# AnneLouisedb/dlwp-benchmark

Measured on AMD Instinct MI355X. Metric: rollout cell-steps/s, higher is better.
Workload: dtype f32 (f16x3: products from two-part f16 splits, 22-bit operands, fp32 accumulate)

## Files before the change

dlwp_benchmark_amd/csrc/fno2d.hip:

```cpp
#include "common.hpp"
#include "spectral_any.hpp"
#include <atomic>
#include <memory>

#ifndef DLWP_GELU8_LIFT
#define DLWP_GELU8_LIFT gelu_erf8
#endif
#ifndef DLWP_GELU8_PROJ
#define DLWP_GELU8_PROJ gelu_erf8
#endif
#ifndef DLWP_GELU8_TRUNK
#define DLWP_GELU8_TRUNK gelu_erf8
#endif

namespace dlwp {
namespace fno {

constexpr int kC = 32;
constexpr int kTrStride = 68;

struct ChanSeg {
  const float* ptr;
  long long bstride;
  int nchan;
// ... 873 lines not shown
        const int c = 4 * s + g;
        *reinterpret_cast<f32x4*>(s_tr + c * kTrStride + 4 * j) =
            *reinterpret_cast<const f32x4*>(x + ((long long)b * kC + c) * HW + pix);
      }
      wave_lds_fence();
      fwd_dft_accumulate<2, KP>(s_tr, tt, w0, lane, yacc);
      wave_lds_fence();
    }
    store_y<2, KP>(ybuf, row, kC, lane, yacc);
  }
}

struct ModesParams {
  const float* ybuf;
  float* zbuf;
  const float2* wt;
  const float2* ef;
  const float2* ei;
  const float* ck;
  float fwd_scale;
  int B, H, M1, M2, KP;
};

__device__ __forceinline__ float2 cfma(float2 a, float2 b, float2 c) {
  return float2{fmaf(a.x, b.x, fmaf(-a.y, b.y, c.x)), fmaf(a.x, b.y, fmaf(a.y, b.x, c.y))};
}

template <int HC, int RG>
__global__ __launch_bounds__(1024) void fno_modes_kernel(const ModesParams p) {
  extern __shared__ __align__(16) float smem[];
  constexpr int C = kC, CP = 32 / RG, CN = C / CP;
  const int ky = blockIdx.x, b = blockIdx.y, tid = threadIdx.x;
  const int lo = tid & 31, hi = tid >> 5;
  const int H = p.H, M1 = p.M1, KP = p.KP;
  float* zb = p.zbuf + (long long)b * H * KP * C;
  if (ky >= p.M2) {
    for (int i = tid; i < H * C; i += 1024) {
      const int o = i & 31, h = i >> 5;
      zb[((long long)h * KP + 2 * ky) * C + o] = 0.f;
      zb[((long long)h * KP + 2 * ky + 1) * C + o] = 0.f;
    }
    return;
  }
  float2* s_ef = reinterpret_cast<float2*>(smem);
  float2* s_ei = s_ef + M1 * H;
  float2* s_part = s_ei + M1 * H;
  float2* s_x = s_part + 16 * M1 * C;
  float2* s_o = s_x + M1 * C;

  float2 yv[HC];
  {
    const float* yb = p.ybuf + (long long)b * H * KP * C;
#pragma unroll
    for (int i = 0; i < HC; ++i) {
      const int h = hi * HC + i;
      if (h < H) {
        yv[i].x = yb[((long long)h * KP + 2 * ky) * C + lo];
        yv[i].y = yb[((long long)h * KP + 2 * ky + 1) * C + lo];
      } else {
        yv[i] = float2{0.f, 0.f};
      }
    }
  }
  for (int i = tid; i < M1 * H; i += 1024) {
    s_ef[i] = p.ef[i];
    s_ei[i] = p.ei[i];
  }
  const int r2 = hi % RG, cpart = hi / RG;
  float2 wreg[CN];
  {
    const float2* w = p.wt + ((long long)ky * M1 + (r2 < M1 ? r2 : 0)) * C * C + (size_t)cpart * CN * C + lo;
#pragma unroll
    for (int c = 0; c < CN; ++c) wreg[c] = w[c * C];
  }
  __syncthreads();
  for (int r = 0; r < M1; ++r) {
    float2 acc = {0.f, 0.f};
#pragma unroll
    for (int i = 0; i < HC; ++i) {
      const int h = hi * HC + i;
      acc = cfma(yv[i], s_ef[r * H + (h < H ? h : 0)], acc);
    }
    acc.x += __shfl_xor(acc.x, 32);
    acc.y += __shfl_xor(acc.y, 32);
    if ((tid & 32) == 0) s_part[((tid >> 6) * M1 + r) * C + lo] = acc;
  }
  __syncthreads();
  for (int i = tid; i < M1 * C; i += 1024) {
    float2 a = s_part[i];
#pragma unroll
    for (int w = 1; w < 16; ++w) {
      const float2 t = s_part[w * M1 * C + i];
      a.x += t.x;
      a.y += t.y;
    }
    s_x[i] = float2{a.x * p.fwd_scale, a.y * p.fwd_scale};
  }
  __syncthreads();
  if (r2 < M1) {
    float2 acc = {0.f, 0.f};
#pragma unroll
    for (int c = 0; c < CN; ++c) acc = cfma(s_x[r2 * C + cpart * CN + c], wreg[c], acc);
    s_part[(cpart * M1 + r2) * C + lo] = acc;
  }
  __syncthreads();
  for (int i = tid; i < M1 * C; i += 1024) {
    float2 a = s_part[i];
#pragma unroll
    for (int cp = 1; cp < CP; ++cp) {
      const float2 t = s_part[cp * M1 * C + i];
      a.x += t.x;
      a.y += t.y;
    }
    s_o[i] = a;
  }
  __syncthreads();
  {
    float2 acc[HC];
#pragma unroll
    for (int i = 0; i < HC; ++i) acc[i] = float2{0.f, 0.f};
    for (int r = 0; r < M1; ++r) {
      const float2 ov = s_o[r * C + lo];
#pragma unroll
      for (int i = 0; i < HC; ++i) {
        const int h = hi * HC + i;
        acc[i] = cfma(ov, s_ei[r * H + (h < H ? h : 0)], acc[i]);
      }
    }
    const float ck = p.ck[ky];
#pragma unroll
    for (int i = 0; i < HC; ++i) {
      const int h = hi * HC + i;
      if (h < H) {
        zb[((long long)h * KP + 2 * ky) * C + lo] = acc[i].x * ck;
        zb[((long long)h * KP + 2 * ky + 1) * C + lo] = acc[i].y * ck;
      }
    }
  }
}

constexpr int kTrunkMaxLayers = 8;
#ifndef DLWP_TRUNK_DFT_BF16
#define DLWP_TRUNK_DFT_BF16 0
#endif
constexpr bool kDftBf16 = DLWP_TRUNK_DFT_BF16 != 0;
#ifndef DLWP_F16_DFT
#define DLWP_F16_DFT 1
#endif
#ifndef DLWP_PREFETCH_EARLY
#define DLWP_PREFETCH_EARLY 0
#endif
constexpr int kTrunkF16Shift = 3;
constexpr float kTrunkF16Up = 16384.0f, kTrunkF16Down = 1.0f / 16384.0f;
constexpr int kSyStride = 528;

struct TrunkParams {
  const float* x;
  float* y;
  const float* ybuf;
  const float* t;
  const float* tt;
  const u32x4* tb;
  const u32x4* ttb;
  const float2* ef;
  const float2* ei;
  const float* ck;
  const u32x4* wsb[kTrunkMaxLayers];
  const float* bias[kTrunkMaxLayers];
  const float2* wt[kTrunkMaxLayers];
  float* xpart;
  float* obuf;
  long long xpart_par, obuf_par;
  unsigned layer0;
  unsigned* xcc_tab;
  unsigned* ctr;
  unsigned epoch;
  float fwd_scale;
  int S, H, L, M1, M2, G, sample0;
  unsigned long long* trace;
  int trace_tid;
  ChanTable in;
  int lift_ns, lift_hid;
  int lift_cin1;
  const float* lift_w1p;
  const float* lift_b1;
  const u32x4* lift_w2b;
  const float* lift_b2;
  const float* lift_tab;
  float lift_up, lift_down, proj_up, proj_down;
  int proj_hid, proj_co, cout;
  const u32x4* proj_w1b;
  const float* proj_b1;
  const float* proj_w2v;
  const float* proj_b2;
  float* out;
  long long out_bstride;
  const float* resid;
  long long resid_bstride;
  const float* r_const;
  const float* r_presc;
  const float* r_prog;
  float* r_out;
  int r_nconst, r_npresc, r_nprog, r_T, r_ctx, r_t0;
  int feed_regs;
  int n_steps;
  int spin_limit, try_limit;
  unsigned* fail_word;
  unsigned* sticky_fails;
};

__device__ __forceinline__ void trunk_group_barrier(unsigned* ctr, unsigned target, int* s_fail, int spin_limit) {
  __builtin_amdgcn_fence(__ATOMIC_RELEASE, "workgroup");
  __builtin_amdgcn_s_waitcnt(0);
  __syncthreads();
  if (threadIdx.x == 0) {
    __hip_atomic_fetch_add(ctr, 1u, __ATOMIC_RELAXED, __HIP_MEMORY_SCOPE_AGENT);
    int spins = 0;
    while ((int)(__hip_atomic_load(ctr, __ATOMIC_RELAXED, __HIP_MEMORY_SCOPE_AGENT) - target) < 0) {
      __builtin_amdgcn_s_sleep(1);
      if (++spins > spin_limit) {
        *s_fail = 1;
        break;
      }
    }
  }
  __syncthreads();
}

__device__ __forceinline__ void trunk_group_arrive(unsigned* ctr) {
  __builtin_amdgcn_fence(__ATOMIC_RELEASE, "workgroup");
  __builtin_amdgcn_s_waitcnt(0);
  __syncthreads();
  if (threadIdx.x == 0) __hip_atomic_fetch_add(ctr, 1u, __ATOMIC_RELAXED, __HIP_MEMORY_SCOPE_AGENT);
}
__device__ __forceinline__ void trunk_group_wait(unsigned* ctr, unsigned target, int* s_fail, int spin_limit) {
  if (threadIdx.x == 0) {
    int spins = 0;
    while ((int)(__hip_atomic_load(ctr, __ATOMIC_RELAXED, __HIP_MEMORY_SCOPE_AGENT) - target) < 0) {
      __builtin_amdgcn_s_sleep(1);
      if (++spins > spin_limit) {
        *s_fail = 1;
        break;
      }
    }
  }
  __syncthreads();
}

__device__ __forceinline__ float ld_sc1(const float* p) {
  return __hip_atomic_load(p, __ATOMIC_RELAXED, __HIP_MEMORY_SCOPE_AGENT);
}
__device__ __forceinline__ void st_sc1(float* p, float v) {
  __hip_atomic_store(p, v, __ATOMIC_RELAXED, __HIP_MEMORY_SCOPE_AGENT);
}

__device__ __forceinline__ void ld4_sc1_x4(const float* base, unsigned o0, unsigned o1, unsigned o2, unsigned o3,
                                           f32x4& v0, f32x4& v1, f32x4& v2, f32x4& v3) {
  asm volatile(
      "s_nop 4\n\t"
      "global_load_dwordx4 %0, %4, %8 sc1\n\t"
      "global_load_dwordx4 %1, %5, %8 sc1\n\t"
      "global_load_dwordx4 %2, %6, %8 sc1\n\t"
      "global_load_dwordx4 %3, %7, %8 sc1\n\t"
      "s_waitcnt vmcnt(0)"
      : "=&v"(v0), "=&v"(v1), "=&v"(v2), "=&v"(v3)
      : "v"(o0), "v"(o1), "v"(o2), "v"(o3), "s"(base)
      : "memory");
}
constexpr unsigned kSentinel = 0x7fc0deadu;
__device__ __forceinline__ bool has_sentinel(const f32x4& v) {
  return __float_as_uint(v[0]) == kSentinel || __float_as_uint(v[1]) == kSentinel ||
         __float_as_uint(v[2]) == kSentinel || __float_as_uint(v[3]) == kSentinel;
}
__device__ __forceinline__ void st4_sc1(const float* base, unsigned off, const f32x4& v) {
  asm volatile("s_nop 4\n\tglobal_store_dwordx4 %0, %1, %2 sc1\n\ts_nop 1" : : "v"(off), "v"(v), "s"(base) : "memory");
}
__device__ __forceinline__ void st4_l2(const float* base, unsigned off, const f32x4& v) {
  asm volatile("s_nop 4\n\tglobal_store_dwordx4 %0, %1, %2\n\ts_nop 1" : : "v"(off), "v"(v), "s"(base) : "memory");
}
__device__ __forceinline__ void st_xchg(float* p, float v, bool fast) {
  if (fast) *p = v;
  else __hip_atomic_store(p, v, __ATOMIC_RELAXED, __HIP_MEMORY_SCOPE_AGENT);
}

__device__ __forceinline__ void lds_barrier() {
  asm volatile("s_waitcnt lgkmcnt(0)\n\ts_barrier" ::: "memory");
}
__device__ __forceinline__ f32x4 shfl_xor4(f32x4 v, int m) {
  return f32x4{__shfl_xor(v[0], m), __shfl_xor(v[1], m), __shfl_xor(v[2], m), __shfl_xor(v[3], m)};
}

__device__ __forceinline__ void rollout_step_io(const TrunkParams& p, int t, long long HW, ChanTable& in, float*& out,
                                                long long& out_bs, const float*& resid, long long& resid_bs) {
  const int T = p.r_T, ctx = p.r_ctx, To = T - ctx;
  const long long prog_bs = (long long)T * p.r_nprog * HW;
  out_bs = (long long)To * p.r_nprog * HW;
  int k = 0;
#pragma unroll
  for (int i = 0; i < 4; ++i) in.seg[i] = ChanSeg{nullptr, 0, 0, 0};
  if (p.r_nconst) in.seg[k++] = ChanSeg{p.r_const, (long long)p.r_nconst * HW, p.r_nconst, 0};
  if (p.r_npresc)
    in.seg[k++] = ChanSeg{p.r_presc + (long long)(t - ctx) * p.r_npresc * HW, (long long)T * p.r_npresc * HW, p.r_npresc * ctx, 0};
  const int f0 = t - ctx;
  const int n_in = (f0 < ctx) ? (ctx - f0 < ctx ? ctx - f0 : ctx) : 0;
  if (n_in > 0) in.seg[k++] = ChanSeg{p.r_prog + (long long)f0 * p.r_nprog * HW, prog_bs, p.r_nprog * n_in, 0};
  if (ctx - n_in > 0) {
    const int fo = f0 + n_in - ctx;
    in.seg[k++] = ChanSeg{p.r_out + (long long)fo * p.r_nprog * HW, out_bs, p.r_nprog * (ctx - n_in), 0};
  }
  if (t - 1 < ctx) { resid = p.r_prog + (long long)(t - 1) * p.r_nprog * HW; resid_bs = prog_bs; }
  else { resid = p.r_out + (long long)(t - 1 - ctx) * p.r_nprog * HW; resid_bs = out_bs; }
  out = p.r_out + (long long)(t - ctx) * p.r_nprog * HW;
}

template <bool F16 = false>
__device__ __forceinline__ void fwd_dft_bf16x6(const float* s_tr, const u32x4* s_ttb, int lane, f32x4 (&yacc)[2]) {
  const int j = lane & 15, g = lane >> 4;
#pragma unroll
  for (int kb = 0; kb < 2; ++kb) {
    u32x4 tb[3];
#pragma unroll
    for (int pp = 0; pp < 3; ++pp) tb[pp] = s_ttb[(kb * 3 + pp) * 64 + lane];
#pragma unroll
    for (int ct = 0; ct < 2; ++ct) {
      const float* src = s_tr + (16 * ct + j) * kTrStride + 32 * kb + 8 * g;
      const f32x4 a0 = *reinterpret_cast<const f32x4*>(src), a1 = *reinterpret_cast<const f32x4*>(src + 4);
      u32x4 xa[3];
#pragma unroll
      for (int i = 0; i < 4; ++i) {
        unsigned hh, mm, ll;
        const float v0 = i < 2 ? a0[2 * i] : a1[2 * i - 4], v1 = i < 2 ? a0[2 * i + 1] : a1[2 * i - 3];
        split_pair_x<F16>(v0, v1, hh, mm, ll);
        xa[0][i] = hh;
        xa[1][i] = mm;
        xa[2][i] = ll;
      }
      if constexpr (F16) {
        yacc[ct] = mfma16x16x32_f16(xa[0], tb[1], yacc[ct]);
        yacc[ct] = mfma16x16x32_f16(xa[1], tb[0], yacc[ct]);
        yacc[ct] = mfma16x16x32_f16(xa[0], tb[2], yacc[ct]);
      } else {
        yacc[ct] = mfma_bf16x6(xa, tb, yacc[ct]);
      }
    }
  }
}

template <int ROWS, int G, bool LL, bool STEP = false, bool F16 = false>
__global__ __launch_bounds__(64 * ROWS, 2) void fno_trunk_kernel(const TrunkParams p) {
  extern __shared__ __align__(16) float smem[];
  constexpr int W = 64, KP = 16, C = kC, NT = 64 * ROWS;
  constexpr bool kDftF16 = F16 && (DLWP_F16_DFT != 0);
  static_assert(!F16 || kDftF16, "f16x3: the skip convolution and the inverse W-DFT share one SCALED accumulator (common.hpp)");
  constexpr bool kDftMx = kDftBf16 || kDftF16;
  const int tid = threadIdx.x, lane = tid & 63, wave = tid >> 6;
  const int j = lane & 15, g = lane >> 4;
  float* s_tr = smem + wave * (C * kTrStride);
  float* s_y = smem + ROWS * C * kTrStride;
  float* s_z = s_y + ROWS * kSyStride;
  float* s_x = s_z + ROWS * KP * C;
  float* s_t = s_x + ROWS * 128;
  float* s_tt = s_t + KP * W;
  int* s_fail = reinterpret_cast<int*>(s_tt + W * KP);
  int* s_fast = s_fail + 1;
  float2* s_ef = reinterpret_cast<float2*>(s_fail + 4);
  float2* s_ei = s_ef + 16 * ROWS;
  u32x4* s_tb = reinterpret_cast<u32x4*>(s_ei + 16 * ROWS);
  u32x4* s_ttb = s_tb + 4 * 3 * 64;
  const int H = p.H, M1 = p.M1, M2 = p.M2, NM = M1 * M2;
  int sample, member;
  {
    const int i = blockIdx.x;
    if ((p.S & 7) == 0) {
      const int slot = i >> 3;
      sample = (i & 7) + 8 * (slot / G);
      member = slot % G;
    } else {
      sample = i / G;
      member = i % G;
    }
  }
  const int h = member * ROWS + wave;
  const long long HW = (long long)H * W;
  const int gs = p.sample0 + sample;
  const long long pix = (long long)h * W + 4 * j;
  unsigned* ctr = p.ctr + sample * 32;
  if (tid == 0) {
    *s_fail = 0;
    *s_fast = 0;
    if (LL) {
      const unsigned xcc = __builtin_amdgcn_s_getreg((20 << 0) | (0 << 6) | (31 << 11)) & 0xFu;
      __hip_atomic_store(p.xcc_tab + sample * 32 + member, ((p.layer0 + 1u) << 4) | xcc, __ATOMIC_RELAXED,
                         __HIP_MEMORY_SCOPE_AGENT);
    }
  }
  for (int i = tid; i < ROWS * KP * C; i += NT) s_z[i] = 0.f;
  for (int i = tid; i < KP * W; i += NT) {
    s_t[i] = p.t[i];
    s_tt[i] = p.tt[i];
  }
  for (int i = tid; i < 16 * ROWS; i += NT) {
    const int r = i / ROWS, hl = i % ROWS;
    s_ef[i] = r < M1 ? p.ef[r * H + member * ROWS + hl] : float2{0.f, 0.f};
    s_ei[i] = r < M1 ? p.ei[r * H + member * ROWS + hl] : float2{0.f, 0.f};
  }
  for (int i = tid; i < 4 * 3 * 64; i += NT) s_tb[i] = p.tb[i];
  for (int i = tid; i < 2 * 3 * 64; i += NT) s_ttb[i] = p.ttb[i];
  lds_barrier();

  int n_stamp = 0;
  const int n_steps = (STEP && p.n_steps > 1) ? p.n_steps : 1;
  f32x4 vfeed = {0.f, 0.f, 0.f, 0.f};
  u32x4 pre_w2[6];
  float pre_w1[8], pre_b1 = 0.f;
  bool staged = false;
  for (int st = 0; st < n_steps; ++st) {
  int tid_o = threadIdx.x;
  asm volatile("" : "+v"(tid_o));
  const int tid = tid_o, lane = tid & 63, wave = tid >> 6, j = lane & 15, g = lane >> 4;
  float* s_tr = smem + wave * (C * kTrStride);
  const int h = member * ROWS + wave;
  const long long pix = (long long)h * W + 4 * j;
  ChanTable in = p.in;
  float* out_p = p.out;
  long long out_bs = p.out_bstride, resid_bs = p.resid_bstride;
  const float* resid_p = p.resid;
  if (STEP && p.n_steps > 1) rollout_step_io(p, p.r_t0 + st, HW, in, out_p, out_bs, resid_p, resid_bs);
  f32x4 vv[2][4];
  if constexpr (STEP) {
    if (p.trace && tid == p.trace_tid && n_stamp < 64) p.trace[blockIdx.x * 64 + n_stamp++] = __builtin_amdgcn_s_memrealtime();
    const int ntile_l = p.lift_hid >> 4, npair = ntile_l >> 1;
    u32x4* l_w2 = reinterpret_cast<u32x4*>(smem);
    float* l_w1 = reinterpret_cast<float*>(l_w2 + npair * 6 * 64);
    float* l_b1 = l_w1 + ntile_l * p.lift_ns * 64;
    if (!staged) {
      for (int i = tid; i < npair * 6 * 64; i += NT) l_w2[i] = p.lift_w2b[i];
      for (int i = tid; i < ntile_l * p.lift_ns * 64; i += NT) l_w1[i] = p.lift_w1p[i];
      for (int i = tid; i < p.lift_hid; i += NT) l_b1[i] = p.lift_b1[i];
    }
    f32x4 xs[4];
    if (p.feed_regs && st > 0) {
      xs[0] = vfeed;
#pragma unroll
      for (int s = 1; s < 4; ++s) xs[s] = f32x4{0.f, 0.f, 0.f, 0.f};
    } else {
#pragma unroll
      for (int s = 0; s < 4; ++s) {
        const float* cp = s < p.lift_ns ? chan_ptr(in, 4 * s + g, gs, (int)HW) : nullptr;
        xs[s] = cp ? *reinterpret_cast<const f32x4*>(cp + pix) : f32x4{0.f, 0.f, 0.f, 0.f};
      }
    }
    f32x4 bias2[2];
    bias2[0] = *reinterpret_cast<const f32x4*>(p.lift_b2 + 4 * g);
    bias2[1] = *reinterpret_cast<const f32x4*>(p.lift_b2 + 16 + 4 * g);
    lds_barrier();
    if (p.trace && tid == p.trace_tid && n_stamp < 64) p.trace[blockIdx.x * 64 + n_stamp++] = __builtin_amdgcn_s_memrealtime();
    bool from_table = false;
    f32x4 xp = {0.f, 0.f, 0.f, 0.f};
#ifndef DLWP_NO_LIFT_TABLE
    if (p.lift_tab) {
      bool inside = true;
#pragma unroll
      for (int q = 0; q < 4; ++q) {
        xp[q] = __shfl(xs[0][q], lane >> 2);
        inside = inside && (fabsf(xp[q]) < (float)kLiftTabRange);
      }
      from_table = __all(inside) != 0;
    }
#endif
    if (from_table) {
      f32x4 vp[2][4];
      lift_from_table(p.lift_tab, xp, lane & 3, vp);
#pragma unroll
      for (int ot = 0; ot < 2; ++ot)
#pragma unroll
        for (int r = 0; r < 4; ++r)
#pragma unroll
          for (int q = 0; q < 4; ++q) vv[ot][r][q] = __shfl(vp[ot][r][q], 4 * j + g);
    } else {
      f32x4 acc2[2][4];
      lift_segment<4, F16>(xs, l_w1, l_b1, l_w2, npair, lane, bias2, acc2, p.lift_ns, p.lift_cin1 != 0, p.lift_up, p.lift_down);
#pragma unroll
      for (int ot = 0; ot < 2; ++ot)
#pragma unroll
        for (int r = 0; r < 4; ++r) vv[ot][r] = f32x4{acc2[ot][0][r], acc2[ot][1][r], acc2[ot][2][r], acc2[ot][3][r]};
    }
    if (p.trace && tid == p.trace_tid && n_stamp < 64) p.trace[blockIdx.x * 64 + n_stamp++] = __builtin_amdgcn_s_memrealtime();
    lds_barrier();
    if (p.trace && tid == p.trace_tid && n_stamp < 64) p.trace[blockIdx.x * 64 + n_stamp++] = __builtin_amdgcn_s_memrealtime();
#pragma unroll
    for (int ot = 0; ot < 2; ++ot)
#pragma unroll
      for (int r = 0; r < 4; ++r)
        *reinterpret_cast<f32x4*>(s_tr + (16 * ot + 4 * g + r) * kTrStride + 4 * j) = vv[ot][r];
    wave_lds_fence();
    f32x4 yacc[2] = {f32x4{0.f, 0.f, 0.f, 0.f}, f32x4{0.f, 0.f, 0.f, 0.f}};
    if constexpr (kDftMx) {
      fwd_dft_bf16x6<kDftF16>(s_tr, s_ttb, lane, yacc);
    } else {
#pragma unroll
      for (int s = 0; s < 16; ++s)
#pragma unroll
        for (int ct = 0; ct < 2; ++ct)
          yacc[ct] = mfma16x16x4(s_tr[(16 * ct + j) * kTrStride + 4 * s + g], s_tt[(4 * s + g) * KP + j], yacc[ct]);
    }
    wave_lds_fence();
#pragma unroll
    for (int ct = 0; ct < 2; ++ct)
      *reinterpret_cast<f32x4*>(s_y + wave * kSyStride + j * C + 16 * ct + 4 * g) = kDftF16 ? yacc[ct] * kTrunkF16Down : yacc[ct];
    if (p.trace && tid == p.trace_tid && n_stamp < 64) p.trace[blockIdx.x * 64 + n_stamp++] = __builtin_amdgcn_s_memrealtime();
  } else {
#pragma unroll
    for (int ot = 0; ot < 2; ++ot)
#pragma unroll
      for (int r = 0; r < 4; ++r)
        vv[ot][r] = *reinterpret_cast<const f32x4*>(p.x + ((long long)gs * C + 16 * ot + 4 * g + r) * HW + pix);
    const float* yr = p.ybuf + ((long long)gs * H + h) * KP * C;
#pragma unroll
    for (int u = 0; u < 2; ++u)
      *reinterpret_cast<f32x4*>(s_y + wave * kSyStride + 4 * lane + 256 * u) =
          *reinterpret_cast<const f32x4*>(yr + 4 * lane + 256 * u);
  }
  constexpr int KS1 = ROWS / 2;
  float a_re[KS1], a_im[KS1];
#pragma unroll
  for (int s = 0; s < KS1; ++s) {
    const int hl = 2 * s + (g >> 1);
    float2 e = {0.f, 0.f};
    if (j < M1) e = s_ef[j * ROWS + hl];
    a_re[s] = (g & 1) ? -e.y : e.x;
    a_im[s] = (g & 1) ? e.x : e.y;
  }
  float a3[8];
#pragma unroll
  for (int s = 0; s < 8; ++s) {
    const int r = 2 * s + (g >> 1);
    float2 e = {0.f, 0.f};
    if (r < M1 && (j >> 1) < ROWS) e = s_ei[r * ROWS + (j >> 1)];
    a3[s] = (j & 1) ? ((g & 1) ? e.x : e.y) : ((g & 1) ? -e.y : e.x);
  }
  const int ks3 = (2 * M1 + 3) / 4;
  const int per = (NM + G - 1) / G;
  const int m_lo = member * per, m_hi = (m_lo + per < NM) ? m_lo + per : NM;
  float* xp_mine0 = p.xpart + ((long long)sample * G + member) * NM * 64;
  const float* xp_grp0 = p.xpart + (long long)sample * G * NM * 64;
  float* ob0 = p.obuf + (long long)sample * NM * 64;
  unsigned target = p.epoch * (unsigned)G;

#define DLWP_STAMP()                                                                                   \
  do {                                                                                                 \
    if (p.trace && tid == p.trace_tid && n_stamp < 64) p.trace[blockIdx.x * 64 + n_stamp++] = __builtin_amdgcn_s_memrealtime(); \
  } while (0)
  DLWP_STAMP();

  for (int l = 0; l < p.L; ++l) {
    const int par = LL ? (int)((p.layer0 + (unsigned)(st * p.L + l)) & 1u) : 0;
    float* xp_mine = xp_mine0 + par * p.xpart_par;
    const float* xp_grp = xp_grp0 + par * p.xpart_par;
    float* ob = ob0 + par * p.obuf_par;
    float* ob_other = ob0 + (par ^ 1) * p.obuf_par;
    if (LL) asm volatile("s_waitcnt vmcnt(0)" ::: "memory");
    const bool fast = LL && (l > 0 || st > 0) && (*s_fast != 0);
    u32x4 wb[2][3];
#pragma unroll
    for (int ot = 0; ot < 2; ++ot)
#pragma unroll
      for (int pp = 0; pp < 3; ++pp) wb[ot][pp] = p.wsb[l][(ot * 3 + pp) * 64 + lane];
    f32x4 bias4[2];
#pragma unroll
    for (int ot = 0; ot < 2; ++ot) bias4[ot] = *reinterpret_cast<const f32x4*>(p.bias[l] + 16 * ot + 4 * g);
    float2 wreg[2][16];
    {
      const int m = m_lo + wave;
      const float2* w = p.wt[l] + ((long long)(m < m_hi ? m : 0) * C + (lane >> 5) * 16) * C + (lane & 31);
#pragma unroll
      for (int cc = 0; cc < 16; ++cc) wreg[0][cc] = w[cc * C];
    }
    lds_barrier();
    DLWP_STAMP();
    for (int ky = wave; ky < M2; ky += ROWS) {
      f32x4 dre[2] = {f32x4{0.f, 0.f, 0.f, 0.f}, f32x4{0.f, 0.f, 0.f, 0.f}}, dim[2] = {dre[0], dre[0]};
#pragma unroll
      for (int s = 0; s < KS1; ++s) {
#pragma unroll
        for (int nt = 0; nt < 2; ++nt) {
          const float b = s_y[(2 * s + (g >> 1)) * kSyStride + (2 * ky + (g & 1)) * C + 16 * nt + j];
          dre[nt] = mfma16x16x4(a_re[s], b, dre[nt]);
          dim[nt] = mfma16x16x4(a_im[s], b, dim[nt]);
        }
      }
      auto publish = [&](auto fastc) {
        constexpr bool FAST = decltype(fastc)::value;
#pragma unroll
        for (int nt = 0; nt < 2; ++nt)
#pragma unroll
          for (int r4 = 0; r4 < 4; ++r4) {
            const int r = 4 * g + r4;
            if (r < M1) {
              float* dst = xp_mine + (long long)(ky * M1 + r) * 64 + 16 * nt + j;
              if constexpr (!LL) {
                st_sc1(dst, dre[nt][r4]);
                st_sc1(dst + 32, dim[nt][r4]);
              } else if constexpr (FAST) {
                dst[0] = dre[nt][r4];
                dst[32] = dim[nt][r4];
              } else {
                __hip_atomic_store(dst, dre[nt][r4], __ATOMIC_RELAXED, __HIP_MEMORY_SCOPE_AGENT);
                __hip_atomic_store(dst + 32, dim[nt][r4], __ATOMIC_RELAXED, __HIP_MEMORY_SCOPE_AGENT);
              }
            }
          }
      };
      if (fast) publish(std::true_type{}); else publish(std::false_type{});
    }
    DLWP_STAMP();
    target += (unsigned)G;
    if (!LL) trunk_group_arrive(ctr);
    f32x4 acc[2][4];
#pragma unroll
    for (int ot = 0; ot < 2; ++ot)
#pragma unroll
      for (int q = 0; q < 4; ++q) acc[ot][q] = F16 ? bias4[ot] * kTrunkF16Up : bias4[ot];
#pragma unroll
    for (int q = 0; q < 4; ++q) {
      u32x4 bx[3];
#pragma unroll
      for (int i = 0; i < 4; ++i) {
        unsigned hh, mm, ll;
        split_pair_x<F16>(vv[i >> 1][2 * (i & 1)][q], vv[i >> 1][2 * (i & 1) + 1][q], hh, mm, ll);
        bx[0][i] = hh;
        bx[1][i] = mm;
        bx[2][i] = ll;
      }
#pragma unroll
      for (int ot = 0; ot < 2; ++ot) acc[ot][q] = mfma_x<F16>(wb[ot], bx, acc[ot][q]);
    }
    if (!LL) trunk_group_wait(ctr, target, s_fail, p.spin_limit);
    DLWP_STAMP();
    {
      const int m = m_lo + wave + ROWS;
      const float2* w = p.wt[l] + ((long long)(m < m_hi ? m : 0) * C + (lane >> 5) * 16) * C + (lane & 31);
#pragma unroll
// ... 151 lines not shown
            s_z[(2 * g + (r4 >> 1)) * (KP * C) + (kDftMx ? o * KP + kq : kq * C + o)] = d[r4] * ckw;
          }
      }
      wave_lds_fence();
    }
    lds_barrier();
    DLWP_STAMP();
    if constexpr (kDftMx) {
      u32x4 za[2][3];
#pragma unroll
      for (int ot = 0; ot < 2; ++ot) {
        f32x4 z0 = {0.f, 0.f, 0.f, 0.f}, z1 = z0;
        if (g < 2) {
          const float* src = s_z + wave * (KP * C) + (16 * ot + j) * KP + 8 * g;
          z0 = *reinterpret_cast<const f32x4*>(src);
          z1 = *reinterpret_cast<const f32x4*>(src + 4);
        }
#pragma unroll
        for (int i = 0; i < 4; ++i) {
          unsigned hh, mm, ll;
          const float v0 = i < 2 ? z0[2 * i] : z1[2 * i - 4], v1 = i < 2 ? z0[2 * i + 1] : z1[2 * i - 3];
          split_pair_x<kDftF16>(v0, v1, hh, mm, ll);
          za[ot][0][i] = hh;
          za[ot][1][i] = mm;
          za[ot][2][i] = ll;
        }
      }
#pragma unroll
      for (int q = 0; q < 4; ++q) {
        u32x4 tb[3];
#pragma unroll
        for (int pp = 0; pp < 3; ++pp) tb[pp] = s_tb[(q * 3 + pp) * 64 + lane];
#pragma unroll
        for (int ot = 0; ot < 2; ++ot) {
          if constexpr (kDftF16) {
            acc[ot][q] = mfma16x16x32_f16(za[ot][0], tb[1], acc[ot][q]);
            acc[ot][q] = mfma16x16x32_f16(za[ot][1], tb[0], acc[ot][q]);
            acc[ot][q] = mfma16x16x32_f16(za[ot][0], tb[2], acc[ot][q]);
          } else {
            acc[ot][q] = mfma_bf16x6(za[ot], tb, acc[ot][q]);
          }
        }
      }
    } else {
      float z[KP / 4][2];
#pragma unroll
      for (int s = 0; s < KP / 4; ++s)
#pragma unroll
        for (int ot = 0; ot < 2; ++ot) z[s][ot] = s_z[wave * (KP * C) + (4 * s + g) * C + 16 * ot + j];
#pragma unroll
      for (int s = 0; s < KP / 4; ++s) {
        const f32x4 tw = *reinterpret_cast<const f32x4*>(s_t + (4 * s + g) * W + 4 * j);
#pragma unroll
        for (int q = 0; q < 4; ++q)
#pragma unroll
          for (int ot = 0; ot < 2; ++ot) acc[ot][q] = mfma16x16x4(z[s][ot], tw[q], acc[ot][q]);
      }
    }
#pragma unroll
    for (int ot = 0; ot < 2; ++ot)
#pragma unroll
      for (int r = 0; r < 4; ++r) {
        vv[ot][r] = f32x4{acc[ot][0][r], acc[ot][1][r], acc[ot][2][r], acc[ot][3][r]};
        if constexpr (F16) vv[ot][r] *= kTrunkF16Down;
      }
    DLWP_STAMP();
    if (l < p.L - 1) {
#pragma unroll
      for (int ot = 0; ot < 2; ++ot) {
        DLWP_GELU8_TRUNK(vv[ot][0], vv[ot][1]);
        DLWP_GELU8_TRUNK(vv[ot][2], vv[ot][3]);
      }
      DLWP_STAMP();
#pragma unroll
      for (int ot = 0; ot < 2; ++ot)
#pragma unroll
        for (int r = 0; r < 4; ++r)
          *reinterpret_cast<f32x4*>(s_tr + (16 * ot + 4 * g + r) * kTrStride + 4 * j) = vv[ot][r];
      wave_lds_fence();
      DLWP_STAMP();
      f32x4 yacc[2] = {f32x4{0.f, 0.f, 0.f, 0.f}, f32x4{0.f, 0.f, 0.f, 0.f}};
      if constexpr (kDftMx) {
        fwd_dft_bf16x6<kDftF16>(s_tr, s_ttb, lane, yacc);
      } else {
#pragma unroll
        for (int s = 0; s < 16; ++s)
#pragma unroll
          for (int ct = 0; ct < 2; ++ct)
            yacc[ct] = mfma16x16x4(s_tr[(16 * ct + j) * kTrStride + 4 * s + g], s_tt[(4 * s + g) * KP + j], yacc[ct]);
      }
      wave_lds_fence();
      DLWP_STAMP();
#pragma unroll
      for (int ct = 0; ct < 2; ++ct)
        *reinterpret_cast<f32x4*>(s_y + wave * kSyStride + j * C + 16 * ct + 4 * g) = kDftF16 ? yacc[ct] * kTrunkF16Down : yacc[ct];
    }
  }
  DLWP_STAMP();
#undef DLWP_STAMP
  if (*s_fail) {
    if (tid == 0 && p.fail_word) {
      atomicOr(p.fail_word, 1u);
      atomicAdd(p.sticky_fails, 1u);
    }
    const float nanv = __uint_as_float(0x7fc00000u);
#pragma unroll
    for (int ot = 0; ot < 2; ++ot)
#pragma unroll
      for (int r = 0; r < 4; ++r) vv[ot][r] = f32x4{nanv, nanv, nanv, nanv};
  }
  if (STEP && p.proj_hid > 0) {
    const int ntile_p = p.proj_hid >> 4;
    const int n_q1 = ntile_p * 3 * 64, n_q2 = ntile_p * p.proj_co * 16;
    u32x4 pq1[6];
    float pq2[2], pqb;
#pragma unroll
    for (int k = 0; k < 6; ++k) {
      const int i = tid + k * NT;
      pq1[k] = p.proj_w1b[i < n_q1 ? i : 0];
    }
#pragma unroll
    for (int k = 0; k < 2; ++k) {
      const int i = tid + k * NT;
      pq2[k] = p.proj_w2v[i < n_q2 ? i : 0];
    }
    pqb = p.proj_b1[tid < p.proj_hid ? tid : 0];
    lds_barrier();
    u32x4* q_w1 = reinterpret_cast<u32x4*>(smem);
    float* q_b1 = reinterpret_cast<float*>(q_w1 + ntile_p * 3 * 64);
    float* q_w2 = q_b1 + p.proj_hid;
#pragma unroll
    for (int k = 0; k < 6; ++k) {
      const int i = tid + k * NT;
      if (i < n_q1) q_w1[i] = pq1[k];
    }
#pragma unroll
    for (int k = 0; k < 2; ++k) {
      const int i = tid + k * NT;
      if (i < n_q2) q_w2[i] = pq2[k];
    }
    if (tid < p.proj_hid) q_b1[tid] = F16 ? pqb * p.proj_up : pqb;
    u32x4 bx[4][3];
#pragma unroll
    for (int q = 0; q < 4; ++q)
#pragma unroll
      for (int i = 0; i < 4; ++i) {
        unsigned hh, mm, ll;
        split_pair_x<F16>(vv[i >> 1][2 * (i & 1)][q], vv[i >> 1][2 * (i & 1) + 1][q], hh, mm, ll);
        bx[q][0][i] = hh;
        bx[q][1][i] = mm;
        bx[q][2][i] = ll;
      }
    lds_barrier();
    auto lift_prefetch = [&]() {
      const int n_w2p = (p.lift_hid >> 5) * 6 * 64, n_w1p = (p.lift_hid >> 4) * p.lift_ns * 64;
#pragma unroll
      for (int k = 0; k < 6; ++k) {
        const int i = tid + k * NT;
        pre_w2[k] = p.lift_w2b[i < n_w2p ? i : 0];
      }
#pragma unroll
      for (int k = 0; k < 8; ++k) {
        const int i = tid + k * NT;
        pre_w1[k] = p.lift_w1p[i < n_w1p ? i : 0];
      }
      pre_b1 = p.lift_b1[tid < p.lift_hid ? tid : 0];
    };
#if DLWP_PREFETCH_EARLY
    if (st + 1 < n_steps) lift_prefetch();
#endif
    f32x4 v = {0.f, 0.f, 0.f, 0.f};
    auto run = [&](auto coc) {
      constexpr int CO = decltype(coc)::value;
      float po[CO][4];
      proj_segment<CO, F16>(bx, q_w1, q_b1, q_w2, ntile_p, lane, po, p.proj_down);
#pragma unroll
      for (int co = 0; co < CO; ++co)
#pragma unroll
        for (int q = 0; q < 4; ++q) {
          float x = po[co][q];
          x += __shfl_xor(x, 16);
          x += __shfl_xor(x, 32);
          if (g == co) v[q] = x;
        }
    };
    if (p.proj_co == 1) run(std::integral_constant<int, 1>{});
    else if (p.proj_co == 2) run(std::integral_constant<int, 2>{});
    else run(std::integral_constant<int, 4>{});
    if (g < p.cout) {
      const float b2 = p.proj_b2[g];
      v += f32x4{b2, b2, b2, b2};
      if (p.feed_regs && st > 0) v += vfeed;
      else if (resid_p) v += *reinterpret_cast<const f32x4*>(resid_p + (long long)gs * resid_bs + (long long)g * HW + pix);
      if (*s_fail) v = f32x4{__uint_as_float(0x7fc00000u), __uint_as_float(0x7fc00000u), __uint_as_float(0x7fc00000u),
                             __uint_as_float(0x7fc00000u)};
      *reinterpret_cast<f32x4*>(out_p + (long long)gs * out_bs + (long long)g * HW + pix) = v;
      if constexpr (F16) {
        const float mag = fabsf(v[0]) + fabsf(v[1]) + fabsf(v[2]) + fabsf(v[3]);
        if (!(mag < 3.0e38f) && p.fail_word) {
          atomicOr(p.fail_word, 2u);
          atomicAdd(p.sticky_fails + 1, 1u);
        }
      }
    }
    if (p.trace && tid == p.trace_tid && n_stamp < 64) p.trace[blockIdx.x * 64 + n_stamp++] = __builtin_amdgcn_s_memrealtime();
    if (st + 1 < n_steps) {
      const int npair_n = p.lift_hid >> 5, n_w2 = npair_n * 6 * 64, n_w1 = (p.lift_hid >> 4) * p.lift_ns * 64;
#if !DLWP_PREFETCH_EARLY
      lift_prefetch();
#endif
      if (p.feed_regs) {
        vfeed = (g < p.cout) ? v : f32x4{0.f, 0.f, 0.f, 0.f};
      } else {
        asm volatile("s_waitcnt vmcnt(0)" ::: "memory");
        __builtin_amdgcn_fence(__ATOMIC_ACQUIRE, "workgroup");
      }
      lds_barrier();
      {
        u32x4* l_w2n = reinterpret_cast<u32x4*>(smem);
        float* l_w1n = reinterpret_cast<float*>(l_w2n + n_w2);
        float* l_b1n = l_w1n + n_w1;
#pragma unroll
        for (int k = 0; k < 6; ++k) {
          const int i = tid + k * NT;
          if (i < n_w2) l_w2n[i] = pre_w2[k];
        }
#pragma unroll
        for (int k = 0; k < 8; ++k) {
          const int i = tid + k * NT;
          if (i < n_w1) l_w1n[i] = pre_w1[k];
        }
        if (tid < p.lift_hid) l_b1n[tid] = pre_b1;
      }
      staged = true;
    }
    continue;
  }
#pragma unroll
  for (int ot = 0; ot < 2; ++ot)
#pragma unroll
    for (int r = 0; r < 4; ++r)
      *reinterpret_cast<f32x4*>(p.y + ((long long)gs * C + 16 * ot + 4 * g + r) * HW + pix) = vv[ot][r];
  }
}

__global__ __launch_bounds__(256) void pack_spectral_kernel(const float2* __restrict__ src, float2* __restrict__ dst,
                                                            int Ci, int Co, int R, int K, int adjoint) {
  const long long total = (long long)Ci * Co * R * K;
  for (long long i = (long long)blockIdx.x * blockDim.x + threadIdx.x; i < total; i += (long long)gridDim.x * blockDim.x) {
    const int ky = (int)(i % K);
    const int r = (int)((i / K) % R);
    const int o = (int)((i / ((long long)K * R)) % Co);
    const int c = (int)(i / ((long long)K * R * Co));
    const float2 v = src[i];
    if (adjoint) dst[(((long long)ky * R + r) * Co + o) * Ci + c] = float2{v.x, -v.y};
    else dst[(((long long)ky * R + r) * Ci + c) * Co + o] = v;
  }
}

struct SpectralCore {
  int H = 0, W = 0, M1 = 0, M2 = 0, KP = 0;
  float fwd_scale = 1.f;
  DevBuf t, tt, ef, ei, ck;
  DevBuf tb, ttb;
  DevBuf tbh, ttbh;

  int32_t build(int H_, int W_, int M1_, int M2_, const int32_t* rows_in, const int32_t* rows_out,
                float fwd, float inv, hipStream_t s) {
    H = H_; W = W_; M1 = M1_; M2 = M2_; fwd_scale = fwd;
    KP = (2 * M2 <= 16) ? 16 : 32;
    DLWP_REQUIRE(2 * M2 <= 32, DLWP_ERR_UNSUPPORTED, "kept rfft columns %d > 16 not supported", M2);
    DLWP_REQUIRE(M2 <= W / 2 + 1 && M1 <= H, DLWP_ERR_INVALID_ARGUMENT, "modes exceed the grid");
    const double two_pi = 6.283185307179586476925286766559;
    std::vector<float> ht((size_t)KP * W, 0.f), htt((size_t)W * KP, 0.f);
    for (int ky = 0; ky < M2; ++ky)
      for (int w = 0; w < W; ++w) {
        const long long m = ((long long)ky * w) % W;
        const double a = two_pi * (double)m / (double)W;
        const float c = (float)std::cos(a), sn = (float)(-std::sin(a));
        ht[(size_t)(2 * ky) * W + w] = c;
        ht[(size_t)(2 * ky + 1) * W + w] = sn;
        htt[(size_t)w * KP + 2 * ky] = c;
        htt[(size_t)w * KP + 2 * ky + 1] = sn;
      }
    std::vector<float> hef((size_t)M1 * H * 2), hei((size_t)M1 * H * 2), hck(M2);
    for (int r = 0; r < M1; ++r)
      for (int h = 0; h < H; ++h) {
        const long long mi = ((long long)rows_in[r] * h) % H, mo = ((long long)rows_out[r] * h) % H;
        const double ai = two_pi * (double)mi / (double)H, ao = two_pi * (double)mo / (double)H;
        hef[((size_t)r * H + h) * 2 + 0] = (float)std::cos(ai);
        hef[((size_t)r * H + h) * 2 + 1] = (float)(-std::sin(ai));
        hei[((size_t)r * H + h) * 2 + 0] = (float)std::cos(ao);
        hei[((size_t)r * H + h) * 2 + 1] = (float)std::sin(ao);
      }
    for (int ky = 0; ky < M2; ++ky) {
      const bool self_conj = (ky == 0) || (W % 2 == 0 && ky == W / 2);
      hck[ky] = (self_conj ? 1.f : 2.f) * inv;
    }
    if (W == 64 && KP == 16) {
      std::vector<uint32_t> htb((size_t)4 * 3 * 64 * 4, 0u), httb((size_t)2 * 3 * 64 * 4, 0u);
      std::vector<uint32_t> htbh(htb.size(), 0u), httbh(httb.size(), 0u);
      for (int l = 0; l < 64; ++l) {
        const int jj0 = l & 15, gg = l >> 4;
        for (int d = 0; d < 4; ++d) {
          for (int q = 0; q < 4; ++q) {
            uint16_t hh[2], mm[2], ll[2];
            for (int e = 0; e < 2; ++e) {
              const int kp = 8 * gg + 2 * d + e;
              split3_host(kp < KP ? ht[(size_t)kp * W + 4 * jj0 + q] : 0.f, hh[e], mm[e], ll[e]);
            }
            {
              uint16_t fh[2], fm[2], fb[2];
              for (int e = 0; e < 2; ++e) {
                const int kp = 8 * gg + 2 * d + e;
                split2_host_f16((kp < KP ? ht[(size_t)kp * W + 4 * jj0 + q] : 0.f) * (float)(1 << kTrunkF16Shift), fh[e], fm[e]);
                fb[e] = f16_times_2048_host(fh[e]);
              }
              htbh[(((size_t)q * 3 + 0) * 64 + l) * 4 + d] = (uint32_t)fh[0] | ((uint32_t)fh[1] << 16);
              htbh[(((size_t)q * 3 + 1) * 64 + l) * 4 + d] = (uint32_t)fm[0] | ((uint32_t)fm[1] << 16);
              htbh[(((size_t)q * 3 + 2) * 64 + l) * 4 + d] = (uint32_t)fb[0] | ((uint32_t)fb[1] << 16);
            }
            htb[(((size_t)q * 3 + 0) * 64 + l) * 4 + d] = (uint32_t)hh[0] | ((uint32_t)hh[1] << 16);
            htb[(((size_t)q * 3 + 1) * 64 + l) * 4 + d] = (uint32_t)mm[0] | ((uint32_t)mm[1] << 16);
            htb[(((size_t)q * 3 + 2) * 64 + l) * 4 + d] = (uint32_t)ll[0] | ((uint32_t)ll[1] << 16);
          }
          for (int kb = 0; kb < 2; ++kb) {
            uint16_t hh[2], mm[2], ll[2];
            for (int e = 0; e < 2; ++e) {
              const int w = 32 * kb + 8 * gg + 2 * d + e;
              split3_host(htt[(size_t)w * KP + jj0], hh[e], mm[e], ll[e]);
            }
            {
              uint16_t fh[2], fm[2], fb[2];
              for (int e = 0; e < 2; ++e) {
                const int w = 32 * kb + 8 * gg + 2 * d + e;
                split2_host_f16(htt[(size_t)w * KP + jj0] * (float)(1 << kTrunkF16Shift), fh[e], fm[e]);
                fb[e] = f16_times_2048_host(fh[e]);
              }
              httbh[(((size_t)kb * 3 + 0) * 64 + l) * 4 + d] = (uint32_t)fh[0] | ((uint32_t)fh[1] << 16);
              httbh[(((size_t)kb * 3 + 1) * 64 + l) * 4 + d] = (uint32_t)fm[0] | ((uint32_t)fm[1] << 16);
              httbh[(((size_t)kb * 3 + 2) * 64 + l) * 4 + d] = (uint32_t)fb[0] | ((uint32_t)fb[1] << 16);
            }
            httb[(((size_t)kb * 3 + 0) * 64 + l) * 4 + d] = (uint32_t)hh[0] | ((uint32_t)hh[1] << 16);
            httb[(((size_t)kb * 3 + 1) * 64 + l) * 4 + d] = (uint32_t)mm[0] | ((uint32_t)mm[1] << 16);
            httb[(((size_t)kb * 3 + 2) * 64 + l) * 4 + d] = (uint32_t)ll[0] | ((uint32_t)ll[1] << 16);
          }
        }
      }
      DLWP_HIP_CHECK(tb.upload(htb.data(), htb.size() * 4, s));
      DLWP_HIP_CHECK(ttb.upload(httb.data(), httb.size() * 4, s));
      DLWP_HIP_CHECK(tbh.upload(htbh.data(), htbh.size() * 4, s));
      DLWP_HIP_CHECK(ttbh.upload(httbh.data(), httbh.size() * 4, s));
      DLWP_HIP_CHECK(hipStreamSynchronize(s));
    }
    DLWP_HIP_CHECK(t.upload(ht.data(), ht.size() * 4, s));
    DLWP_HIP_CHECK(tt.upload(htt.data(), htt.size() * 4, s));
    DLWP_HIP_CHECK(ef.upload(hef.data(), hef.size() * 4, s));
    DLWP_HIP_CHECK(ei.upload(hei.data(), hei.size() * 4, s));
    DLWP_HIP_CHECK(ck.upload(hck.data(), hck.size() * 4, s));
    DLWP_HIP_CHECK(hipStreamSynchronize(s));
    return DLWP_OK;
  }
  size_t modes_lds_bytes() const { return (size_t)(2 * M1 * H + 18 * M1 * kC) * sizeof(float2); }
};

static void pack_spectral(std::vector<float>& dst, const float* w, int Ci, int Co, int M1blk, int M2,
                          int M1tot, int row_off) {
  for (int c = 0; c < Ci; ++c)
    for (int o = 0; o < Co; ++o)
      for (int r = 0; r < M1blk; ++r)
        for (int ky = 0; ky < M2; ++ky) {
          const size_t src = ((((size_t)c * Co + o) * M1blk + r) * M2 + ky) * 2;
          const size_t d = ((((size_t)ky * M1tot + (r + row_off)) * Ci + c) * Co + o) * 2;
          dst[d] = w[src];
          dst[d + 1] = w[src + 1];
        }
}

static int grid_rows(int nrow, int waves_per_block) {
  int blocks = (nrow + waves_per_block - 1) / waves_per_block;
  const int cap = 256 * 8;
  return blocks < cap ? (blocks > 0 ? blocks : 1) : cap;
}

template <class K>
static hipError_t allow_lds(K kernel, size_t bytes) {
  if (bytes <= 48 * 1024) return hipSuccess;
// ... 1425 lines not shown
```

Measured before the change: 2.137 billion.

## Vote on lift-table use per step and stage lift weights only when needed

When a lift lookup table exists, each wave now checks whether its inputs fall inside the table range and publishes a block-wide flag in shared memory. The block stages the lift MLP weights into LDS and runs the exact path only if some wave needs it. Otherwise it skips the weight staging, the end-of-step prefetch/store and one or two barriers. This is meant to cut per-step global loads, LDS writes and block synchronisation in the rollout loop. The cost is an extra barrier to read the vote, plus double-buffered flag bookkeeping that adds complexity to the control flow.

```diff
diff --git a/dlwp_benchmark_amd/csrc/fno2d.hip b/dlwp_benchmark_amd/csrc/fno2d.hip
--- a/dlwp_benchmark_amd/csrc/fno2d.hip
+++ b/dlwp_benchmark_amd/csrc/fno2d.hip
@@ -1049,6 +1049,16 @@
 #endif
 constexpr int kTrunkF16Shift = 3;
 constexpr float kTrunkF16Up = 16384.0f, kTrunkF16Down = 1.0f / 16384.0f;
+#if defined(DLWP_LIFT_STAGE_ALWAYS) || defined(DLWP_NO_LIFT_TABLE)
+constexpr bool kLiftVote = false;
+#else
+constexpr bool kLiftVote = true;
+#endif
+#ifdef DLWP_LIFT_GATHER_EARLY
+constexpr bool kLiftGatherEarly = true;
+#else
+constexpr bool kLiftGatherEarly = false;
+#endif
 constexpr int kSyStride = 528;
 
 struct TrunkParams {
@@ -1260,6 +1270,7 @@
   float* s_tt = s_t + KP * W;
   int* s_fail = reinterpret_cast<int*>(s_tt + W * KP);
   int* s_fast = s_fail + 1;
+  int* s_lflag = s_fail + 2;
   float2* s_ef = reinterpret_cast<float2*>(s_fail + 4);
   float2* s_ei = s_ef + 16 * ROWS;
   u32x4* s_tb = reinterpret_cast<u32x4*>(s_ei + 16 * ROWS);
@@ -1285,6 +1296,7 @@
   if (tid == 0) {
     *s_fail = 0;
     *s_fast = 0;
+    s_lflag[0] = s_lflag[1] = 0;
     if (LL) {
       const unsigned xcc = __builtin_amdgcn_s_getreg((20 << 0) | (0 << 6) | (31 << 11)) & 0xFu;
       __hip_atomic_store(p.xcc_tab + sample * 32 + member, ((p.layer0 + 1u) << 4) | xcc, __ATOMIC_RELAXED,
@@ -1308,8 +1320,6 @@
   int n_stamp = 0;
   const int n_steps = (STEP && p.n_steps > 1) ? p.n_steps : 1;
   f32x4 vfeed = {0.f, 0.f, 0.f, 0.f};
-  u32x4 pre_w2[6];
-  float pre_w1[8], pre_b1 = 0.f;
   bool staged = false;
   for (int st = 0; st < n_steps; ++st) {
   int tid_o = threadIdx.x;
@@ -1330,11 +1340,21 @@
     u32x4* l_w2 = reinterpret_cast<u32x4*>(smem);
     float* l_w1 = reinterpret_cast<float*>(l_w2 + npair * 6 * 64);
     float* l_b1 = l_w1 + ntile_l * p.lift_ns * 64;
-    if (!staged) {
+    auto lift_stage = [&]() {
       for (int i = tid; i < npair * 6 * 64; i += NT) l_w2[i] = p.lift_w2b[i];
       for (int i = tid; i < ntile_l * p.lift_ns * 64; i += NT) l_w1[i] = p.lift_w1p[i];
       for (int i = tid; i < p.lift_hid; i += NT) l_b1[i] = p.lift_b1[i];
-    }
+    };
+    auto lift_stage_voted = [&]() {
+#pragma unroll 1
+      for (int i = tid; i < npair * 6 * 64; i += NT) l_w2[i] = p.lift_w2b[i];
+#pragma unroll 1
+      for (int i = tid; i < ntile_l * p.lift_ns * 64; i += NT) l_w1[i] = p.lift_w1p[i];
+#pragma unroll 1
+      for (int i = tid; i < p.lift_hid; i += NT) l_b1[i] = p.lift_b1[i];
+    };
+    const bool vote = kLiftVote && p.lift_tab != nullptr;
+    if (!vote && !staged) lift_stage();
     f32x4 xs[4];
     if (p.feed_regs && st > 0) {
       xs[0] = vfeed;
@@ -1350,12 +1370,9 @@
     f32x4 bias2[2];
     bias2[0] = *reinterpret_cast<const f32x4*>(p.lift_b2 + 4 * g);
     bias2[1] = *reinterpret_cast<const f32x4*>(p.lift_b2 + 16 + 4 * g);
-    lds_barrier();
-    if (p.trace && tid == p.trace_tid && n_stamp < 64) p.trace[blockIdx.x * 64 + n_stamp++] = __builtin_amdgcn_s_memrealtime();
     bool from_table = false;
     f32x4 xp = {0.f, 0.f, 0.f, 0.f};
-#ifndef DLWP_NO_LIFT_TABLE
-    if (p.lift_tab) {
+    auto lift_pick = [&]() {
       bool inside = true;
 #pragma unroll
       for (int q = 0; q < 4; ++q) {
@@ -1363,9 +1380,8 @@
         inside = inside && (fabsf(xp[q]) < (float)kLiftTabRange);
       }
       from_table = __all(inside) != 0;
-    }
-#endif
-    if (from_table) {
+    };
+    auto lift_gather = [&]() {
       f32x4 vp[2][4];
       lift_from_table(p.lift_tab, xp, lane & 3, vp);
 #pragma unroll
@@ -1374,17 +1390,57 @@
         for (int r = 0; r < 4; ++r)
 #pragma unroll
           for (int q = 0; q < 4; ++q) vv[ot][r][q] = __shfl(vp[ot][r][q], 4 * j + g);
-    } else {
+    };
+    auto lift_exact = [&]() {
       f32x4 acc2[2][4];
       lift_segment<4, F16>(xs, l_w1, l_b1, l_w2, npair, lane, bias2, acc2, p.lift_ns, p.lift_cin1 != 0, p.lift_up, p.lift_down);
 #pragma unroll
       for (int ot = 0; ot < 2; ++ot)
 #pragma unroll
         for (int r = 0; r < 4; ++r) vv[ot][r] = f32x4{acc2[ot][0][r], acc2[ot][1][r], acc2[ot][2][r], acc2[ot][3][r]};
-    }
-    if (p.trace && tid == p.trace_tid && n_stamp < 64) p.trace[blockIdx.x * 64 + n_stamp++] = __builtin_amdgcn_s_memrealtime();
-    lds_barrier();
-    if (p.trace && tid == p.trace_tid && n_stamp < 64) p.trace[blockIdx.x * 64 + n_stamp++] = __builtin_amdgcn_s_memrealtime();
+    };
+#define DLWP_LIFT_STAMP()                                                                              \
+  do {                                                                                                 \
+    if (p.trace && tid == p.trace_tid && n_stamp < 64) p.trace[blockIdx.x * 64 + n_stamp++] = __builtin_amdgcn_s_memrealtime(); \
+  } while (0)
+    if (vote) {
+      lift_pick();
+      if (!from_table) s_lflag[st & 1] = 1;
+    }
+    if (kLiftGatherEarly && vote && from_table) {
+      lift_gather();
+      DLWP_LIFT_STAMP();
+      lds_barrier();
+      DLWP_LIFT_STAMP();
+      const bool fallback = __builtin_amdgcn_readfirstlane(s_lflag[st & 1]) != 0;
+      if (tid == 0) s_lflag[(st + 1) & 1] = 0;
+      if (fallback) {
+        lift_stage_voted();
+        lds_barrier();
+        lds_barrier();
+      }
+      DLWP_LIFT_STAMP();
+    } else {
+      bool weights_used = true;
+      if (vote) {
+        DLWP_LIFT_STAMP();
+        lds_barrier();
+        weights_used = __builtin_amdgcn_readfirstlane(s_lflag[st & 1]) != 0;
+        if (tid == 0) s_lflag[(st + 1) & 1] = 0;
+      }
+      if (vote && weights_used) lift_stage_voted();
+      if (weights_used) lds_barrier();
+      DLWP_LIFT_STAMP();
+#if defined(DLWP_LIFT_STAGE_ALWAYS) && !defined(DLWP_NO_LIFT_TABLE)
+      if (p.lift_tab) lift_pick();
+#endif
+      if (!from_table) lift_exact();
+      else if (!kLiftVote || !kLiftGatherEarly) lift_gather();
+      if (!vote) DLWP_LIFT_STAMP();
+      if (weights_used) lds_barrier();
+      DLWP_LIFT_STAMP();
+    }
+#undef DLWP_LIFT_STAMP
 #pragma unroll
     for (int ot = 0; ot < 2; ++ot)
 #pragma unroll
@@ -1842,6 +1898,8 @@
         bx[q][2][i] = ll;
       }
     lds_barrier();
+    u32x4 pre_w2[6];
+    float pre_w1[8], pre_b1 = 0.f;
     auto lift_prefetch = [&]() {
       const int n_w2p = (p.lift_hid >> 5) * 6 * 64, n_w1p = (p.lift_hid >> 4) * p.lift_ns * 64;
 #pragma unroll
@@ -1857,7 +1915,7 @@
       pre_b1 = p.lift_b1[tid < p.lift_hid ? tid : 0];
     };
 #if DLWP_PREFETCH_EARLY
-    if (st + 1 < n_steps) lift_prefetch();
+    if (st + 1 < n_steps && !(kLiftVote && p.lift_tab != nullptr)) lift_prefetch();
 #endif
     f32x4 v = {0.f, 0.f, 0.f, 0.f};
     auto run = [&](auto coc) {
@@ -1896,17 +1954,22 @@
     if (p.trace && tid == p.trace_tid && n_stamp < 64) p.trace[blockIdx.x * 64 + n_stamp++] = __builtin_amdgcn_s_memrealtime();
     if (st + 1 < n_steps) {
       const int npair_n = p.lift_hid >> 5, n_w2 = npair_n * 6 * 64, n_w1 = (p.lift_hid >> 4) * p.lift_ns * 64;
+      auto feed_next = [&]() {
+        if (p.feed_regs) {
+          vfeed = (g < p.cout) ? v : f32x4{0.f, 0.f, 0.f, 0.f};
+        } else {
+          asm volatile("s_waitcnt vmcnt(0)" ::: "memory");
+          __builtin_amdgcn_fence(__ATOMIC_ACQUIRE, "workgroup");
+        }
+      };
+      if (kLiftVote && p.lift_tab != nullptr) {
+        feed_next();
+      } else {
 #if !DLWP_PREFETCH_EARLY
-      lift_prefetch();
+        lift_prefetch();
 #endif
-      if (p.feed_regs) {
-        vfeed = (g < p.cout) ? v : f32x4{0.f, 0.f, 0.f, 0.f};
-      } else {
-        asm volatile("s_waitcnt vmcnt(0)" ::: "memory");
-        __builtin_amdgcn_fence(__ATOMIC_ACQUIRE, "workgroup");
-      }
-      lds_barrier();
-      {
+        feed_next();
+        lds_barrier();
         u32x4* l_w2n = reinterpret_cast<u32x4*>(smem);
         float* l_w1n = reinterpret_cast<float*>(l_w2n + n_w2);
         float* l_b1n = l_w1n + n_w1;
@@ -1921,8 +1984,8 @@
           if (i < n_w1) l_w1n[i] = pre_w1[k];
         }
         if (tid < p.lift_hid) l_b1n[tid] = pre_b1;
-      }
-      staged = true;
+        staged = true;
+      }
     }
     continue;
   }
```

New measurement: 2.274 billion, median of 6. 1.06x the previous value.
